# HengyiWang/MorpheuS

Hardware: AMD Instinct MI355X
Metric: rays/sec (fwd+bwd, 128 samples/ray) (higher is better)
Workload: dtype f32 (exact 3 x bf16 operand split on the bf16 MFMA pipe, fp32 accumulate)

## Files before the change

include/morpheus_hip.h:

```cpp
#ifndef MORPHEUS_HIP_H
#define MORPHEUS_HIP_H

#include <stdint.h>

#ifdef __cplusplus
extern "C" {
#endif

#define MH_OK 0
#define MH_ERR_ARG 1
#define MH_ERR_LAUNCH 2
#define MH_ERR_OVERFLOW 3

#define MH_ABI_VERSION 9
#define MH_MAX_LEVELS 32
#define MH_TILE 32

int mh_abi_version(void);
const char *mh_status_string(int status);

int mh_grid_encode_fwd(const float *x, const float *emb, const int32_t *offsets_host,
                       const int32_t *res_host, float *out, int64_t M, int32_t L, int32_t n_levels,
                       float bound, int32_t group, void *stream);
int mh_grid_encode_bwd(const float *grad, const float *x, const float *emb,
                       const int32_t *offsets_host, const int32_t *res_host, float *grad_emb,
                       float *grad_x, int64_t M, int32_t L, int32_t n_levels, float bound, void *stream);

int64_t mh_grid_bin_workspace_ints(void);
int32_t mh_grid_bin_bricks(void);
int32_t mh_grid_bin_index_ints(void);
int mh_grid_bin_points(const float *x, int64_t M, float bound, int32_t *workspace, int32_t *perm,
                       int32_t *brick_start, void *stream);
int mh_grid_encode_bwd_binned(const float *grad, const float *x, const float *emb,
                              const int32_t *offsets_host, const int32_t *res_host, const int32_t *perm,
                              const int32_t *brick_start, float *grad_emb, int64_t *emb_acc, float *grad_x, int32_t accumulate_dx,
                              int64_t M, int32_t L, int32_t n_levels, float bound, const uint32_t *gmax_bits, void *stream);
int mh_grid_encode_fwd_binned(const float *x, const float *emb, const int32_t *offsets_host, const int32_t *res_host,
                              const int32_t *perm, const int32_t *brick_start, float *out, int64_t M, int32_t L,
                              int32_t n_levels, float bound, void *stream);
int64_t mh_grid_stage_min_points(int64_t set);
int mh_grid_bwd_layout(const int32_t *res_host, int32_t L, int32_t *cbase, int32_t *stride, int32_t *rows);

int mh_grid_general_fwd(const float *x, const float *emb, const int32_t *offsets_host, const int32_t *res_host, float *out,
                        int64_t M, int32_t L, int32_t n_levels, int32_t C, int32_t gridtype, int32_t align_corners,
                        int32_t interp, float bound, void *stream);
int mh_grid_general_bwd(const float *grad, const float *x, const float *emb, const int32_t *offsets_host,
                        const int32_t *res_host, float *grad_emb, int64_t *emb_acc, float *grad_x, int64_t M, int32_t L,
                        int32_t n_levels, int32_t C, int32_t gridtype, int32_t align_corners, int32_t interp, float bound,
                        void *stream);
int mh_grid_grad_tv(const float *x, const float *emb, const int32_t *offsets_host, const int32_t *res_host, float *grad_emb,
                    int64_t *emb_acc, float weight, int64_t M, int32_t L, int32_t C, int32_t gridtype, int32_t align_corners,
                    int32_t normalized, float bound, void *stream);
int mh_grid_grad_wd(const float *emb, const int32_t *offsets_host, float *grad_emb, float weight, int32_t L, int32_t C,
                    void *stream);

int mh_composite_fwd(const float *sigma, const float *t_starts, const float *t_ends, const float *rgb,
                     const int32_t *ray_start, const int32_t *ray_cnt, float *weights, float *opacity,
                     float *depth, float *color, int32_t N, void *stream);
int mh_composite_bwd(const float *sigma, const float *t_starts, const float *t_ends, const float *rgb,
                     const int32_t *ray_start, const int32_t *ray_cnt, const float *weights,
                     const float *g_weights, const float *g_opacity, const float *g_depth,
                     const float *g_color, float *d_sigma, float *d_rgb, int32_t N, void *stream);

int mh_generate_rays(float fx, float fy, float cx, float cy, const float *c2w_host, int32_t H, int32_t W,
                     float *rays_o, float *rays_d, void *stream);
int mh_sample_uniform(const float *rays_o, const float *rays_d, const float *jitter, int32_t N, int32_t S,
                      float bound, int32_t *ray_idx, float *t_starts, float *t_ends, float *xyz,
                      int32_t *ray_start, int32_t *ray_cnt, void *stream);

int mh_rays_sample_uniform(float fx, float fy, float cx, float cy, const float *c2w_host, int32_t H, int32_t W,
                           const int32_t *pix, const float *jitter, int32_t N, int32_t S, float bound,
                           float *rays_o, float *rays_d, int32_t *ray_idx, float *t_starts, float *t_ends,
                           float *xyz, int32_t *ray_start, int32_t *ray_cnt, void *stream);

int32_t mh_march_cap(float step, float bound);
int mh_march_slots(const float *rays_o, const float *rays_d, const float *jitter, int32_t N, float step, float bound,
                   int32_t R, const uint8_t *binary, int32_t cap, int32_t *ray_cnt, float *slot_ts, float *slot_te,
                   int32_t *overflow, void *stream);
int mh_march_pack(const int32_t *ray_start, const int32_t *ray_cnt, const float *slot_ts, const float *slot_te, int32_t N,
                  int32_t cap, int32_t *ray_idx, float *t_starts, float *t_ends, void *stream);

int mh_visibility_mask(const float *values, int32_t alpha_form, const float *t_starts, const float *t_ends,
                       const int32_t *ray_start, const int32_t *ray_cnt, int32_t N, int64_t M, float early_stop_eps,
                       const float *alpha_thre, uint8_t *keep, int32_t *kept_cnt, void *stream);
int mh_visibility_pack(const uint8_t *keep, const float *t_starts, const float *t_ends, const int32_t *ray_start,
                       const int32_t *ray_cnt, const int32_t *new_start, int32_t N, int64_t M, int64_t M_out,
                       int32_t *out_ray_idx, float *out_t_starts, float *out_t_ends, int32_t *src_index, void *stream);

int mh_fd_taps(const float *x, const float *topo, int32_t topo_dim, float eps, float bound, int64_t M, float *taps,
               float *topo6, void *stream);
int mh_fd_taps_bwd(const float *x, const float *g_taps, const float *g_topo6, int32_t topo_dim, float eps, float bound,
                   int64_t M, float *g_x, float *g_topo, void *stream);
int mh_fd_normal_fwd(const float *sdf6, float eps, int64_t M, float *normal, float *raw, void *stream);
int mh_fd_normal_bwd(const float *sdf6, const float *g_normal, const float *g_raw, float eps, int64_t M, float *g_sdf6,
                     void *stream);
int mh_sample_positions(const float *rays_o, const float *rays_d, const int32_t *ray_idx, const float *t_starts,
                        const float *t_ends, int64_t M, float *xyz, void *stream);
int mh_multicode_fwd(const float *t, const float *v0, const float *v1, const float *v2, int32_t s0, int32_t s1, int32_t s2,
                     int32_t C, int32_t F, float *out, void *stream);
int mh_multicode_bwd(const float *t, const float *g_out, float *g0, float *g1, float *g2, int32_t s0, int32_t s1, int32_t s2,
                     int32_t C, int32_t F, void *stream);
int mh_sdf_losses_fwd(const float *pred_sdf, const float *t_starts, const float *t_ends, const int32_t *ray_idx,
                      const float *rays_depth, const float *rays_mask, float trunc, int64_t M, const int32_t *n_valid,
                      float *sums, void *stream);
int mh_sdf_losses_bwd(const float *pred_sdf, const float *t_starts, const float *t_ends, const int32_t *ray_idx,
                      const float *rays_depth, const float *rays_mask, float trunc, int64_t M, const int32_t *n_valid,
                      const float *sums, const float *g_fs, const float *g_sl, float *g_pred, void *stream);
int mh_sample_positions_bwd(const float *g_xyz, const float *t_starts, const float *t_ends, const int32_t *ray_start,
                            const int32_t *ray_cnt, int32_t N, float *g_o, float *g_d, void *stream);

int64_t mh_mlp_tiles(int64_t M);
int64_t mh_warp_acts_floats(int64_t M);
int64_t mh_warp_dpre_floats(int64_t M);
int64_t mh_warp_wpack_floats(void);
int64_t mh_warp_wpackT_floats(void);
int mh_warp_fwd(const float *x, const int32_t *slot, const float *bias0_d, const float *bias0_t,
                const float *wpack_d, const float *wpack_t, const float *bias_d, const float *bias_t,
                int32_t n_bands, float *out_deform, float *out_topo, float *acts, int64_t M, void *stream);
int64_t mh_field_w3_bytes(void);
int mh_field_fwd_b3(const float *xc, const float *feat_s, const float *feat_c, const float *topo, const void *w3,
                    const float *bias, const float *beta, int32_t n_bands, int32_t with_color, float *sdf, float *sigma,
                    float *albedo, float *acts, int64_t M, void *stream);
// ... 274 lines not shown
```

morpheus_amd/csrc/hashgrid.hip:

```cpp
#include "common.h"
#include "wave.h"
#include <stdlib.h>
#include <algorithm>
#include <atomic>
#include <cmath>

#pragma clang fp contract(off)

struct GridMeta {
    int32_t offsets[MH_MAX_LEVELS + 1];
    int32_t res[MH_MAX_LEVELS];
};

struct Corner8 {
    uint32_t row[8];
    float w[8];
};

__device__ __forceinline__ uint32_t grid_row(uint32_t cx, uint32_t cy, uint32_t cz, uint32_t res, uint32_t T,
                                             bool dense, bool pow2) {
    uint32_t idx;
    if (dense) {
        idx = cx + cy * res + cz * res * res;
        return idx;
// ... 280 lines not shown
    const int t = threadIdx.x;
    int32_t *work_start = brick_start + NBRK + 2;
    int loc[PER], locw[PER], s = 0, sw = 0;
#pragma unroll
    for (int k = 0; k < PER; k++) {
        const int i = t * PER + k;
        loc[k] = i <= NBRK ? brick_cnt[i] : 0;
        locw[k] = i < NBRK ? (loc[k] + chunk - 1) / chunk : 0;
        s += loc[k];
        sw += locw[k];
    }
    part[t] = s;
    partw[t] = sw;
    __syncthreads();
    for (int o = 1; o < 1024; o <<= 1) {
        const int v = t >= o ? part[t - o] : 0;
        const int vw = t >= o ? partw[t - o] : 0;
        __syncthreads();
        part[t] += v;
        partw[t] += vw;
        __syncthreads();
    }
    int run = part[t] - s, runw = partw[t] - sw;
#pragma unroll
    for (int k = 0; k < PER; k++) {
        const int i = t * PER + k;
        if (i <= NBRK) {
            brick_start[i] = run;
            work_start[i] = runw;
        }
        run += loc[k];
        runw += locw[k];
    }
    if (t == 1023) brick_start[NBRK + 1] = part[1023], brick_start[BRK_CHUNK_WORD] = chunk;
}

__global__ __launch_bounds__(256) void bin_scatter_kernel(const float *__restrict__ x, int64_t M, int64_t chunk, float bound,
                                                          float two_bound, const int32_t *__restrict__ block_off,
                                                          const int32_t *__restrict__ brick_start, int32_t *__restrict__ perm) {
    __shared__ int cur[NBRK + 1];
    for (int i = threadIdx.x; i <= NBRK; i += 256) cur[i] = brick_start[i] + block_off[(int64_t)blockIdx.x * (NBRK + 1) + i];
    __syncthreads();
    const int64_t p0 = (int64_t)blockIdx.x * chunk, p1 = min(p0 + chunk, M);
    for (int64_t p = p0 + threadIdx.x; p < p1; p += 256) {
        const int slot = atomicAdd(&cur[brick_of(x, p, bound, two_bound)], 1);
        perm[slot] = (int32_t)p;
    }
}

__global__ __launch_bounds__(256) void absmax_kernel(const float *__restrict__ g, int64_t n, uint32_t *__restrict__ out) {
    uint32_t m = 0;
    const int64_t stride = (int64_t)gridDim.x * blockDim.x;
    const int64_t n4 = n >> 2;
    const f32x4 *g4 = reinterpret_cast<const f32x4 *>(g);
    for (int64_t i = (int64_t)blockIdx.x * blockDim.x + threadIdx.x; i < n4; i += stride) {
        const f32x4 v = g4[i];
        m = max(max(m, __float_as_uint(fabsf(v[0]))), __float_as_uint(fabsf(v[1])));
        m = max(max(m, __float_as_uint(fabsf(v[2]))), __float_as_uint(fabsf(v[3])));
    }
    for (int64_t i = 4 * n4 + (int64_t)blockIdx.x * blockDim.x + threadIdx.x; i < n; i += stride) m = max(m, __float_as_uint(fabsf(g[i])));
    m = wave_max(m);
    if ((threadIdx.x & 63) == 0 && m) atomicMax(out, m);
}

#define FX_BITS 40
#define FX_MAGIC 6755399441055744.0
#define FX_MAGIC_BITS 0x4338000000000000ULL
#define FX_LIMIT 1099511627776.0f
__device__ __forceinline__ void fx_scales(uint32_t maxbits, float &to_fx, float &from_fx) {
    int e = (int)(maxbits >> 23) + 1;
    e = max(e, 60);
    e = min(e, 254);
    to_fx = __uint_as_float((uint32_t)(127 + FX_BITS + 127 - e) << 23);
    from_fx = __uint_as_float((uint32_t)(127 - FX_BITS - 127 + e) << 23);
}

#define BRK_THREADS 1024
constexpr int BRK_PIPE = 2;
constexpr int BRK_STAGE = 1;
constexpr int BRK_STAGE_UNROLL = 8;
constexpr int BRK_STAGE_MIN_POINTS = 1 << 20;
constexpr int BRK_STAGE_MIN = 96;

__device__ __forceinline__ int brk_div(int j, int m) { return (int)(((uint32_t)j * (uint32_t)m) >> 16); }

__device__ __forceinline__ bool brk_find_item(const int32_t *__restrict__ brick_start, int w, int *item) {
    const int32_t *work_start = brick_start + NBRK + 2;
    constexpr int PER = NBRK / BRK_THREADS;
    const int b0 = PER * (int)threadIdx.x;
    int ws[PER + 1], bs[PER + 1];
    const int chunk = brick_start[BRK_CHUNK_WORD];
#pragma unroll
    for (int k = 0; k <= PER; k++) ws[k] = work_start[b0 + k], bs[k] = brick_start[b0 + k];
    bool mine = false;
#pragma unroll
    for (int k = 0; k < PER; k++)
        if (ws[k] <= w && w < ws[k + 1]) {
            const int first = bs[k] + (w - ws[k]) * chunk;
            item[0] = b0 + k, item[1] = first, item[2] = min(first + chunk, bs[k + 1]), mine = true;
        }
    return __syncthreads_or(mine) != 0;
}

struct BrickLevel {
    uint32_t res, T, my, mz, mask, sel;
    bool dense, pow2;
    int nn, base, lo[3];
    const float2 *tab;
};

__device__ __forceinline__ BrickLevel brk_level(const GridMeta &meta, const BrickMeta &bm, const float2 *__restrict__ emb, int l,
                                                int brick) {
    BrickLevel v;
    v.res = (uint32_t)meta.res[l];
    v.T = (uint32_t)(meta.offsets[l + 1] - meta.offsets[l]);
    v.dense = (uint64_t)v.res * v.res * v.res <= (uint64_t)v.T;
    v.pow2 = (v.T & (v.T - 1)) == 0;
    v.my = v.dense ? v.res : 2654435761u, v.mz = v.dense ? v.res * v.res : 805459861u;
    v.mask = v.pow2 ? v.T - 1 : 0xffffffffu, v.sel = v.dense ? 0xffffffffu : 0u;
    v.nn = bm.n[l], v.base = bm.lds_off[l];
    const int bxyz[3] = {brick % BRK, (brick / BRK) % BRK, brick / (BRK * BRK)};
#pragma unroll
    for (int d = 0; d < 3; d++) {
        const float pos = fminf(fmaxf(fmaf((float)bxyz[d] / (float)BRK, (float)v.res, -0.5f), 0.0f), (float)(v.res - 1));
        v.lo[d] = (int)floorf(pos);
    }
    v.tab = emb + meta.offsets[l];
    return v;
}

template <bool ZERO>
__device__ __forceinline__ void brk_stage_rows(const BrickLevel &v, int sub, char *lds, int row0, int stride, int z0 = 0, int z1 = 0) {
    const int n3 = v.nn * v.nn * v.nn, m = (65536 + v.nn - 1) / v.nn;
    for (int j0 = sub; j0 < n3; j0 += 64 * BRK_STAGE_UNROLL) {
        float2 r[BRK_STAGE_UNROLL];
#pragma unroll
        for (int u = 0; u < BRK_STAGE_UNROLL; u++) {
            const int j = min(j0 + 64 * u, n3 - 1);
            const int t = brk_div(j, m), jz = brk_div(t, m);
            const int jx = j - t * v.nn, jy = t - jz * v.nn;
            const uint32_t cx = min((uint32_t)(v.lo[0] + jx), v.res - 1), ym = min((uint32_t)(v.lo[1] + jy), v.res - 1) * v.my,
                           zm = min((uint32_t)(v.lo[2] + jz), v.res - 1) * v.mz;
            uint32_t row = ((cx + ym + zm) & v.sel) | ((cx ^ ym ^ zm) & v.mask & ~v.sel);
            if (__builtin_expect(!v.dense && !v.pow2, 0)) row %= v.T;
            r[u] = v.tab[row];
        }
#pragma unroll
        for (int u = 0; u < BRK_STAGE_UNROLL; u++) {
            const int j = j0 + 64 * u;
            if (j < n3) {
                *reinterpret_cast<float2 *>(lds + row0 + j * stride) = r[u];
                if (ZERO) *reinterpret_cast<long long *>(lds + z0 + j * stride) = 0, *reinterpret_cast<long long *>(lds + z1 + j * stride) = 0;
            }
        }
    }
}

__device__ __forceinline__ void brk_zero_sums(int n3, int sub, char *lds, int stride, int z0, int z1) {
    for (int j = sub; j < n3; j += 64)
        *reinterpret_cast<long long *>(lds + z0 + j * stride) = 0, *reinterpret_cast<long long *>(lds + z1 + j * stride) = 0;
}

__global__ __launch_bounds__(BRK_THREADS, 8) void grid_fwd_brick_kernel(const float *__restrict__ x, const float2 *__restrict__ emb,
                                                                         GridMeta meta, BrickMeta bm,
                                                                         const int32_t *__restrict__ perm,
                                                                         const int32_t *__restrict__ brick_start,
                                                                         float2 *__restrict__ out, int L, int n_levels, float bound,
                                                                         float two_bound) {
    __shared__ long long val[BRK_NODES_MAX];
    __shared__ int item[3];
    const int l = threadIdx.x & 15, sub = threadIdx.x >> 4;
    constexpr int PPI = BRK_THREADS / 16;
    if (!brk_find_item(brick_start, blockIdx.x, item)) {
        const int s = (int)blockIdx.x - brick_start[NBRK + 2 + NBRK];
        const int first = brick_start[NBRK] + s * BRK_CHUNK_SMALL, stop = min(first + BRK_CHUNK_SMALL, brick_start[NBRK + 1]);
        for (int i = first + sub; i < stop; i += PPI) out[(int64_t)perm[i] * L + l] = make_float2(0.f, 0.f);
        return;
    }
    const int brick = item[0], start = item[1], end = item[2];
    const bool lev_on = l < n_levels;
    const BrickLevel lv = brk_level(meta, bm, emb, l, brick);
    if (lev_on) brk_stage_rows<false>(lv, sub, reinterpret_cast<char *>(val), 8 * lv.base, 8);
    __syncthreads();
    const int last = end - 1;
    int p_cur = perm[min(start + sub, last)], p_nxt = perm[min(start + sub + PPI, last)];
    float xv[3] = {x[(int64_t)p_cur * 3 + 0], x[(int64_t)p_cur * 3 + 1], x[(int64_t)p_cur * 3 + 2]};
    for (int i = start + sub; i < end; i += PPI) {
        const int p_nn = perm[min(i + 2 * PPI, last)];
        const float xn[3] = {x[(int64_t)p_nxt * 3 + 0], x[(int64_t)p_nxt * 3 + 1], x[(int64_t)p_nxt * 3 + 2]};
        float2 r = make_float2(0.f, 0.f);
        if (lev_on) {
            uint32_t g[3];
            float f[3];
            grid_locate(xv, bound, two_bound, lv.res, g, f);
            const uint32_t g1[3] = {min(g[0] + 1, lv.res - 1), min(g[1] + 1, lv.res - 1), min(g[2] + 1, lv.res - 1)};
            const int lx[2] = {(int)g[0] - lv.lo[0], (int)g1[0] - lv.lo[0]}, ly[2] = {(int)g[1] - lv.lo[1], (int)g1[1] - lv.lo[1]},
                      lz[2] = {(int)g[2] - lv.lo[2], (int)g1[2] - lv.lo[2]};
            float2 v[8];
#pragma unroll
            for (int c = 0; c < 8; c++)
                v[c] = *reinterpret_cast<const float2 *>(
                    &val[lv.base + lx[c & 1] + __mul24(lv.nn, ly[(c >> 1) & 1] + __mul24(lv.nn, lz[(c >> 2) & 1]))]);
#pragma unroll
            for (int c = 0; c < 8; c++) {
                const float w = ((c & 1) ? f[0] : 1.f - f[0]) * ((c & 2) ? f[1] : 1.f - f[1]) * ((c & 4) ? f[2] : 1.f - f[2]);
                r.x = fmaf(w, v[c].x, r.x);
                r.y = fmaf(w, v[c].y, r.y);
            }
        }
        out[(int64_t)p_cur * L + l] = r;
        p_cur = p_nxt, p_nxt = p_nn;
        xv[0] = xn[0], xv[1] = xn[1], xv[2] = xn[2];
    }
}

template <int NEED_DX, bool STAGED>
__global__ __launch_bounds__(BRK_THREADS, STAGED ? 4 : 8) void grid_bwd_brick_kernel(
    const float2 *__restrict__ grad, const float *__restrict__ x, const float2 *__restrict__ emb, GridMeta meta, BrickMeta bm,
    const int32_t *__restrict__ perm, const int32_t *__restrict__ brick_start, long long *__restrict__ emb_acc, int acc_shift,
    float *__restrict__ grad_x, int L, int n_levels, float bound, float two_bound, const uint32_t *__restrict__ gmax_bits) {
    constexpr int ACC_WORDS = STAGED ? 16 * BRK_ACC_ROWS : 2 * BRK_NODES_MAX;
    __shared__ long long acc[ACC_WORDS];
    char *accb = reinterpret_cast<char *>(acc);
    __shared__ int item[3];
    if (!brk_find_item(brick_start, blockIdx.x, item)) return;
    const int brick = item[0], start = item[1], end = item[2];
    const bool staged = STAGED && end - start >= BRK_STAGE_MIN;
    if (!STAGED)
        for (int i = threadIdx.x; i < BRK_NODES_MAX; i += BRK_THREADS) acc[2 * i] = 0, acc[2 * i + 1] = 0;
    float to_fx, from_fx;
    fx_scales(*gmax_bits, to_fx, from_fx);
    to_fx = ldexpf(to_fx, -acc_shift);
    const float fx_lim = ldexpf(FX_LIMIT, -acc_shift);
    const int l = threadIdx.x & 15, sub = threadIdx.x >> 4;
    const bool lev_on = l < n_levels;
    const BrickLevel lv = brk_level(meta, bm, emb, l, brick);
    const uint32_t res = lv.res, T = lv.T;
    const bool dense = lv.dense, pow2 = lv.pow2;
    const int nn = lv.nn, base = lv.base;
    const int lo[3] = {lv.lo[0], lv.lo[1], lv.lo[2]};
    const float2 *tab = lv.tab;
    const int stride = STAGED ? bm.stride : 16;
    const int cb0 = STAGED ? bm.cbase[0][l] : 16 * base, cb1 = STAGED ? bm.cbase[1][l] : cb0 + 8, cb2 = STAGED ? bm.cbase[2][l] : 0;
    const int d1 = cb1 - cb0, d2 = cb2 - cb0;
    if (STAGED && lev_on) {
        if (staged) brk_stage_rows<true>(lv, sub, accb, cb2, stride, cb0, cb1);
        else brk_zero_sums(nn * nn * nn, sub, accb, stride, cb0, cb1);
    }
    static_assert(MH_MAX_LEVELS >= 16, "the brick kernels run on 16-level grids (L == 16 is checked by the launchers)");
    __shared__ int flush_par[16][16];
    if (threadIdx.x < 16) {
        int *fp = flush_par[l];
        fp[0] = nn, fp[1] = (65536 + nn - 1) / nn, fp[2] = base, fp[3] = lo[0], fp[4] = lo[1], fp[5] = lo[2];
        fp[6] = (int)(res - 1), fp[7] = (int)lv.my, fp[8] = (int)lv.mz, fp[9] = (int)lv.mask, fp[10] = (int)lv.sel, fp[11] = (int)T;
        fp[12] = (int)(!dense && !pow2), fp[13] = meta.offsets[l], fp[14] = cb0, fp[15] = cb1;
    }
    __syncthreads();
    constexpr int PPI = BRK_THREADS / 16;
    const int end_r = start + ((end - start + PPI - 1) / PPI) * PPI;
    int magic_hi, magic_lo;
    asm("s_mov_b32 %0, 0x43380000" : "=s"(magic_hi));
    asm("s_mov_b32 %0, 0" : "=s"(magic_lo));
    const double magic = __longlong_as_double(((long long)magic_hi << 32) | (unsigned)magic_lo);
    const int last = end - 1;
    constexpr int PIPE = (NEED_DX && !STAGED) ? 0 : BRK_PIPE;
    int p_cur = 0, p_nxt = 0;
    float xv[3] = {0.f, 0.f, 0.f};
    float2 gr = make_float2(0.f, 0.f);
    if (PIPE == 2) {
        p_cur = perm[min(start + sub, last)];
        p_nxt = perm[min(start + sub + PPI, last)];
#pragma unroll
        for (int d = 0; d < 3; d++) xv[d] = x[(int64_t)p_cur * 3 + d];
        gr = grad[(int64_t)p_cur * L + l];
    }
    const float inv_2b = 1.0f / two_bound;
    for (int i = start + sub; i < end_r; i += PPI) {
        const bool live = i < end;
        if (PIPE == 0) p_cur = perm[min(i, last)];
        const int64_t p = p_cur;
        int p_nn = 0;
        float xn[3] = {0.f, 0.f, 0.f};
        float2 grn = make_float2(0.f, 0.f);
        if (PIPE == 2) {
            p_nn = perm[min(i + 2 * PPI, last)];
#pragma unroll
            for (int d = 0; d < 3; d++) xn[d] = x[(int64_t)p_nxt * 3 + d];
            grn = grad[(int64_t)p_nxt * L + l];
        } else {
#pragma unroll
            for (int d = 0; d < 3; d++) xv[d] = x[p * 3 + d];
            gr = grad[p * L + l];
        }
        float gx_old[3] = {0.f, 0.f, 0.f};
        if (NEED_DX == 2 && l == 0) {
#pragma unroll
            for (int d = 0; d < 3; d++) gx_old[d] = grad_x[p * 3 + d];
        }
        float dx[3] = {0.f, 0.f, 0.f};
        if (live && lev_on) {
            uint32_t g[3];
            float f[3];
            grid_locate(xv, bound, two_bound, res, g, f);
            const uint32_t g1[3] = {min(g[0] + 1, res - 1), min(g[1] + 1, res - 1), min(g[2] + 1, res - 1)};
            const int lx0 = (int)g[0] - lo[0], ly0 = (int)g[1] - lo[1], lz0 = (int)g[2] - lo[2];
            const int lx1 = (int)g1[0] - lo[0], ly1 = (int)g1[1] - lo[1], lz1 = (int)g1[2] - lo[2];
            const double gxd = (double)__builtin_amdgcn_fmed3f(gr.x * to_fx, -fx_lim, fx_lim),
                         gyd = (double)__builtin_amdgcn_fmed3f(gr.y * to_fx, -fx_lim, fx_lim);
            int slot[8];
#pragma unroll
            for (int c = 0; c < 8; c++) {
                const float w = ((c & 1) ? f[0] : 1.f - f[0]) * ((c & 2) ? f[1] : 1.f - f[1]) * ((c & 4) ? f[2] : 1.f - f[2]);
                const int li = ((c & 1) ? lx1 : lx0) + __mul24(nn, ((c & 2) ? ly1 : ly0) + __mul24(nn, (c & 4) ? lz1 : lz0));
                slot[c] = cb0 + __mul24(li, stride);
                const double wd = (double)w;
                const unsigned long long qx = (unsigned long long)__double_as_longlong(__builtin_fma(wd, gxd, magic)) - FX_MAGIC_BITS;
                const unsigned long long qy = (unsigned long long)__double_as_longlong(__builtin_fma(wd, gyd, magic)) - FX_MAGIC_BITS;
                atomicAdd(reinterpret_cast<unsigned long long *>(accb + slot[c]), qx);
                atomicAdd(reinterpret_cast<unsigned long long *>(accb + slot[c] + d1), qy);
            }
            if (NEED_DX) {
                float2 v[8];
                if (staged) {
#pragma unroll
                    for (int c = 0; c < 8; c++) v[c] = *reinterpret_cast<const float2 *>(accb + slot[c] + d2);
                } else {
                    uint32_t row[8];
                    grid_rows8(g, g1, res, T, dense, pow2, row);
#pragma unroll
                    for (int c = 0; c < 8; c++) v[c] = tab[row[c]];
                }
                grid_ddx(v, f, gr, (float)res, dx);
            }
        }
        if (NEED_DX) {
            const float sx = sum16(dx[0]), sy = sum16(dx[1]), sz = sum16(dx[2]);
            if (live && l == 0) {
                grad_x[p * 3 + 0] = gx_old[0] + sx * inv_2b;
                grad_x[p * 3 + 1] = gx_old[1] + sy * inv_2b;
                grad_x[p * 3 + 2] = gx_old[2] + sz * inv_2b;
            }
        }
        if (PIPE == 2) {
            p_cur = p_nxt, p_nxt = p_nn;
            xv[0] = xn[0], xv[1] = xn[1], xv[2] = xn[2], gr = grn;
        }
    }
    __syncthreads();
    {
        int total = 0;
        if (n_levels > 0) {
            const int n_last = bm.n[n_levels - 1];
            total = bm.lds_off[n_levels - 1] + n_last * n_last * n_last;
        }
        for (int j = threadIdx.x; j < total; j += BRK_THREADS) {
            int lev = 0;
            if (STAGED) {
#pragma unroll
                for (int k = 1; k < 16; k++) lev += (k < n_levels && j >= bm.lds_off[k]) ? 1 : 0;
            }
            const int a0 = STAGED ? flush_par[lev][14] + (j - flush_par[lev][2]) * stride : 16 * j;
            const int a1 = STAGED ? flush_par[lev][15] + (j - flush_par[lev][2]) * stride : 16 * j + 8;
            const long long qx = *reinterpret_cast<const long long *>(accb + a0), qy = *reinterpret_cast<const long long *>(accb + a1);
            if (qx == 0 && qy == 0) continue;
            if (!STAGED) {
#pragma unroll
                for (int k = 1; k < 16; k++) lev += (k < n_levels && j >= bm.lds_off[k]) ? 1 : 0;
            }
            const int *fp = flush_par[lev];
            const int n = fp[0], m = fp[1], jl = j - fp[2];
            const int t = brk_div(jl, m), jz = brk_div(t, m);
            const int jx = jl - t * n, jy = t - jz * n;
            const uint32_t rmax = (uint32_t)fp[6];
            const uint32_t cx = min((uint32_t)(fp[3] + jx), rmax), ym = min((uint32_t)(fp[4] + jy), rmax) * (uint32_t)fp[7],
                           zm = min((uint32_t)(fp[5] + jz), rmax) * (uint32_t)fp[8];
            const uint32_t sel = (uint32_t)fp[10];
            uint32_t row = ((cx + ym + zm) & sel) | ((cx ^ ym ^ zm) & (uint32_t)fp[9] & ~sel);
            if (__builtin_expect(fp[12] != 0, 0)) row %= (uint32_t)fp[11];
            unsigned long long *ga = reinterpret_cast<unsigned long long *>(emb_acc + ((size_t)fp[13] + row) * 2);
            atomicAdd(ga + 0, (unsigned long long)qx);
            atomicAdd(ga + 1, (unsigned long long)qy);
        }
    }
}

__global__ void grid_acc_finalize_kernel(const long long *__restrict__ emb_acc, float *__restrict__ grad_emb, int64_t n, int acc_shift,
                                         const uint32_t *__restrict__ gmax_bits) {
    float to_fx, from_fx;
    fx_scales(*gmax_bits, to_fx, from_fx);
    const double scale = (double)from_fx * (double)(1LL << acc_shift);
    for (int64_t i = (int64_t)blockIdx.x * blockDim.x + threadIdx.x; i < n; i += (int64_t)gridDim.x * blockDim.x) {
        const long long a = emb_acc[i];
        if (a != 0) grad_emb[i] += (float)((double)a * scale);
    }
}

static int fill_meta(GridMeta &m, const int32_t *offsets_host, const int32_t *res_host, int L) {
    if (!offsets_host || !res_host || L < 1 || L > MH_MAX_LEVELS) return MH_ERR_ARG;
    for (int i = 0; i <= L; i++) m.offsets[i] = offsets_host[i];
    for (int i = 0; i < L; i++) {
        m.res[i] = res_host[i];
        if (res_host[i] < 2 || offsets_host[i + 1] <= offsets_host[i]) return MH_ERR_ARG;
    }
    return MH_OK;
}

extern "C" int mh_grid_encode_fwd(const float *x, const float *emb, const int32_t *offsets_host,
                                  const int32_t *res_host, float *out, int64_t M, int32_t L, int32_t n_levels,
                                  float bound, int32_t group, void *stream) {
    if (M == 0) return MH_OK;
    if (!x || !emb || !out || M < 0 || n_levels < 0 || n_levels > L || !(bound > 0.f) || group < 1) return MH_ERR_ARG;
    GridMeta meta;
    int st = fill_meta(meta, offsets_host, res_host, L);
    if (st) return st;
    if (group == 6 && M % 6 == 0) {
        const int64_t n_groups = M / 6;
        const int64_t gblocks = (n_groups * L + 255) / 256;
        if (gblocks > 0x7fffffffLL) return MH_ERR_ARG;
        hipLaunchKernelGGL(grid_fwd_grouped_kernel<6>, dim3((unsigned)gblocks), dim3(256), 0, mh_stream(stream), x,
                           reinterpret_cast<const float2 *>(emb), meta, reinterpret_cast<float2 *>(out), n_groups, (int)L,
                           (int)n_levels, bound, 2.0f * bound);
        MH_CHECK_LAUNCH();
        return MH_OK;
    }
    const int64_t threads = M * L;
    const int64_t blocks = (threads + 255) / 256;
    if (blocks > 0x7fffffffLL) return MH_ERR_ARG;
    hipLaunchKernelGGL(grid_fwd_kernel, dim3((unsigned)blocks), dim3(256), 0, mh_stream(stream), x,
                       reinterpret_cast<const float2 *>(emb), meta, reinterpret_cast<float2 *>(out), M, (int)L, (int)n_levels,
                       bound, 2.0f * bound);
    MH_CHECK_LAUNCH();
    return MH_OK;
}

extern "C" int mh_grid_encode_bwd(const float *grad, const float *x, const float *emb, const int32_t *offsets_host,
                                  const int32_t *res_host, float *grad_emb, float *grad_x, int64_t M, int32_t L,
                                  int32_t n_levels, float bound, void *stream) {
    if (M == 0) return MH_OK;
    if (!grad || !x || !emb || !grad_emb || M < 0 || n_levels < 0 || n_levels > L || !(bound > 0.f)) return MH_ERR_ARG;
    if (grad_x && L != 16) return MH_ERR_ARG;
    GridMeta meta;
    int st = fill_meta(meta, offsets_host, res_host, L);
    if (st) return st;
    const int64_t threads = M * L;
    const int64_t blocks = (threads + 255) / 256;
    if (blocks > 0x7fffffffLL) return MH_ERR_ARG;
    if (grad_x)
        hipLaunchKernelGGL(grid_bwd_kernel<true>, dim3((unsigned)blocks), dim3(256), 0, mh_stream(stream),
                           reinterpret_cast<const float2 *>(grad), x, reinterpret_cast<const float2 *>(emb), meta,
                           grad_emb, grad_x, M, (int)L, (int)n_levels, bound, 2.0f * bound);
    else
        hipLaunchKernelGGL(grid_bwd_kernel<false>, dim3((unsigned)blocks), dim3(256), 0, mh_stream(stream),
                           reinterpret_cast<const float2 *>(grad), x, reinterpret_cast<const float2 *>(emb), meta,
                           grad_emb, grad_x, M, (int)L, (int)n_levels, bound, 2.0f * bound);
    MH_CHECK_LAUNCH();
// ... 19 lines not shown
    G = G < 8 ? 8 : (G > BIN_BLOCKS ? BIN_BLOCKS : G);
    const int64_t chunk = (M + G - 1) / G;
    int32_t *block_hist = workspace, *brick_cnt = workspace + (int64_t)BIN_BLOCKS * (NBRK + 1);
    hipLaunchKernelGGL(bin_hist_kernel, dim3((unsigned)G), dim3(256), 0, mh_stream(stream), x, M, chunk, bound, 2.0f * bound,
                       block_hist);
    hipLaunchKernelGGL(bin_colscan_kernel, dim3((NBRK + 1 + 255) / 256), dim3(256), 0, mh_stream(stream), block_hist,
                       (int)G, brick_cnt);
    hipLaunchKernelGGL(bin_rowscan_kernel, dim3(1), dim3(1024), 0, mh_stream(stream), brick_cnt, brick_start,
                       M >= g_stage_min_points.load(std::memory_order_relaxed) ? BRK_CHUNK_LARGE : BRK_CHUNK_SMALL);
    hipLaunchKernelGGL(bin_scatter_kernel, dim3((unsigned)G), dim3(256), 0, mh_stream(stream), x, M, chunk, bound,
                       2.0f * bound, block_hist, brick_start, perm);
    MH_CHECK_LAUNCH();
    return MH_OK;
}

static int fill_brick_meta(BrickMeta &bm, const int32_t *res_host, int L) {
    bm = BrickMeta{};
    int off = 0;
    for (int l = 0; l < L; l++) {
        const int n = (res_host[l] + BRK - 1) / BRK + 2;
        bm.n[l] = n;
        bm.lds_off[l] = off;
        off += n * n * n;
    }
    return off > BRK_NODES_MAX ? MH_ERR_ARG : MH_OK;
}

static int brick_layout_linear(BrickMeta &bm) {
    for (int k = 0; k < 3; k++)
        for (int l = 0; l < 16; l++) bm.cbase[k][l] = 8 * (3 * bm.lds_off[l] + k);
    bm.stride = 24;
    return (24 * (bm.lds_off[15] + bm.n[15] * bm.n[15] * bm.n[15]) + 127) / 128;
}

static int brick_layout(BrickMeta &bm) {
    int sz[16], col[3][16], h[16] = {}, order[48];
    bool used[3][16] = {};
    for (int l = 0; l < 16; l++) sz[l] = bm.n[l] * bm.n[l] * bm.n[l];
    for (int i = 0; i < 48; i++) order[i] = i;
    std::stable_sort(order, order + 48, [&](int a, int b) { return sz[a % 16] > sz[b % 16]; });
    for (int i = 0; i < 48; i++) {
        const int k = order[i] / 16, l = order[i] % 16;
        int best = -1;
        for (int c = 0; c < 16; c++)
            if (!used[k][c] && (best < 0 || h[c] < h[best])) best = c;
        used[k][best] = true, col[k][l] = best, h[best] += sz[l];
    }
    for (bool moved = true; moved;) {
        moved = false;
        for (int k = 0; k < 3; k++)
            for (int a = 0; a < 16; a++)
                for (int b = a + 1; b < 16; b++) {
                    const int ca = col[k][a], cb = col[k][b], d = sz[a] - sz[b];
                    if (std::max(h[ca] - d, h[cb] + d) < std::max(h[ca], h[cb]))
                        h[ca] -= d, h[cb] += d, col[k][a] = cb, col[k][b] = ca, moved = true;
                }
    }
    const int rows = *std::max_element(h, h + 16);
    if (rows > BRK_ACC_ROWS) return brick_layout_linear(bm);
    int top[16] = {};
    for (int k = 0; k < 3; k++)
        for (int l = 0; l < 16; l++) {
            const int c = col[k][l];
            bm.cbase[k][l] = 128 * top[c] + 8 * c;
            top[c] += sz[l];
        }
    bm.stride = 128;
    return rows;
}

extern "C" int mh_grid_bwd_layout(const int32_t *res_host, int32_t L, int32_t *cbase, int32_t *stride, int32_t *rows) {
    if (!res_host || !cbase || !stride || !rows || L != 16) return MH_ERR_ARG;
    for (int l = 0; l < L; l++)
        if (res_host[l] < 2) return MH_ERR_ARG;
    BrickMeta bm;
    if (int st = fill_brick_meta(bm, res_host, L)) return st;
    *rows = brick_layout(bm);
    *stride = bm.stride;
    for (int k = 0; k < 3; k++)
        for (int l = 0; l < 16; l++) cbase[16 * k + l] = bm.cbase[k][l];
    return MH_OK;
}

extern "C" int mh_grid_encode_fwd_binned(const float *x, const float *emb, const int32_t *offsets_host,
                                         const int32_t *res_host, const int32_t *perm, const int32_t *brick_start, float *out,
                                         int64_t M, int32_t L, int32_t n_levels, float bound, void *stream) {
    if (M == 0) return MH_OK;
    if (!x || !emb || !out || !perm || !brick_start || M < 0 || M > 0x7fffffffLL || n_levels < 0 || n_levels > L || L != 16 ||
        !(bound > 0.f))
        return MH_ERR_ARG;
    GridMeta meta;
    int st = fill_meta(meta, offsets_host, res_host, L);
    if (st) return st;
    BrickMeta bm;
    if ((st = fill_brick_meta(bm, res_host, L))) return st;
    const unsigned work_items = (unsigned)(NBRK + M / BRK_CHUNK_SMALL + 1);
    hipLaunchKernelGGL(grid_fwd_brick_kernel, dim3(work_items), dim3(BRK_THREADS), 0, mh_stream(stream), x,
                       reinterpret_cast<const float2 *>(emb), meta, bm, perm, brick_start, reinterpret_cast<float2 *>(out), (int)L,
                       (int)n_levels, bound, 2.0f * bound);
    MH_CHECK_LAUNCH();
    return MH_OK;
}

extern "C" int mh_grid_encode_bwd_binned(const float *grad, const float *x, const float *emb, const int32_t *offsets_host,
                                         const int32_t *res_host, const int32_t *perm, const int32_t *brick_start,
                                         float *grad_emb, int64_t *emb_acc, float *grad_x, int32_t accumulate_dx, int64_t M,
                                         int32_t L, int32_t n_levels, float bound, const uint32_t *gmax_bits, void *stream) {
    if (M == 0) return MH_OK;
    if (!grad || !x || !emb || !grad_emb || !emb_acc || !perm || !brick_start || M < 0 || n_levels < 0 || n_levels > L || L != 16 ||
        !(bound > 0.f))
        return MH_ERR_ARG;
    GridMeta meta;
    int st = fill_meta(meta, offsets_host, res_host, L);
    if (st) return st;
    BrickMeta bm;
    if ((st = fill_brick_meta(bm, res_host, L))) return st;
    const bool staged = BRK_STAGE && grad_x && M >= g_stage_min_points.load(std::memory_order_relaxed);
    if (staged) brick_layout(bm);
    const unsigned work_items = (unsigned)(NBRK + M / BRK_CHUNK_SMALL + 1);
    int acc_shift = 0;
    while (acc_shift < 40 && (double)M * 8.0 > std::ldexp(1.0, 62 - FX_BITS + acc_shift)) acc_shift++;
    const int64_t n_acc = (int64_t)offsets_host[L] * 2;
    if (!mh_zero_async(emb_acc, sizeof(int64_t) * (size_t)n_acc, mh_stream(stream))) return MH_ERR_LAUNCH;
    const uint32_t *gmax = gmax_bits;
    if (!gmax) {
        uint32_t *own = reinterpret_cast<uint32_t *>(const_cast<int32_t *>(brick_start)) + (2 * NBRK + 4);
        if (!mh_zero_async(own, sizeof(uint32_t), mh_stream(stream))) return MH_ERR_LAUNCH;
        hipLaunchKernelGGL(absmax_kernel, dim3(1024), dim3(256), 0, mh_stream(stream), grad, M * (int64_t)L * 2, own);
        gmax = own;
    }
#define BRK_LAUNCH(DXMODE, STG)                                                                                                \
    hipLaunchKernelGGL((grid_bwd_brick_kernel<DXMODE, STG>), dim3(work_items), dim3(BRK_THREADS), 0, mh_stream(stream),       \
                       reinterpret_cast<const float2 *>(grad), x, reinterpret_cast<const float2 *>(emb), meta, bm, perm,     \
                       brick_start, reinterpret_cast<long long *>(emb_acc), acc_shift, grad_x, (int)L, (int)n_levels, bound,          \
                       2.0f * bound, gmax)
    if (grad_x && accumulate_dx) {
        if (staged) BRK_LAUNCH(2, true); else BRK_LAUNCH(2, false);
    } else if (grad_x) {
        if (!mh_zero_async(grad_x, sizeof(float) * 3 * (size_t)M, mh_stream(stream))) return MH_ERR_LAUNCH;
        if (staged) BRK_LAUNCH(1, true); else BRK_LAUNCH(1, false);
    } else {
        BRK_LAUNCH(0, false);
    }
#undef BRK_LAUNCH
    MH_CHECK_LAUNCH();
    hipLaunchKernelGGL(grid_acc_finalize_kernel, dim3((unsigned)std::min<int64_t>((n_acc + 255) / 256, 4096)), dim3(256), 0,
                       mh_stream(stream), reinterpret_cast<const long long *>(emb_acc), grad_emb, n_acc, acc_shift, gmax);
    MH_CHECK_LAUNCH();
    return MH_OK;
}
```

morpheus_amd/ops.py:

```python
from __future__ import annotations

import ctypes
import math
import os
from typing import Optional, Sequence

import numpy as np
import torch

from . import _lib
from ._lib import check, launch, ptr, require_gpu, stream
from .packing import field_joint_packer, field_packer, warp_joint_packer, warp_packer



class KernelTimer:

    def __init__(self):
        self.enabled = False
        self.records = {}
        self._pool, self._used = [], 0

    def reset(self, enabled: bool):
        self.enabled, self.records, self._used = enabled, {}, 0
# ... 56 lines not shown
            key = (len(a),) + tuple(int(v) for v in a)
            hit = _I32_CACHE.get(key)
            if hit is None:
                arr = np.ascontiguousarray(a, dtype=np.int32)
                arr.setflags(write=False)
                hit = _I32_CACHE[key] = (arr, arr.ctypes.data_as(ctypes.c_void_p))
            _I32_CACHE[k2] = hit
            return hit
        key = None
    elif isinstance(a, np.ndarray) and a.dtype == np.int32 and a.ndim == 1 and a.size <= 64:
        key = (a.size,) + tuple(a.tolist())
    else:
        key = None
    if key is not None:
        hit = _I32_CACHE.get(key)
        if hit is None:
            arr = np.ascontiguousarray(a, dtype=np.int32)
            arr.setflags(write=False)
            hit = _I32_CACHE[key] = (arr, arr.ctypes.data_as(ctypes.c_void_p))
        return hit
    a = np.ascontiguousarray(a, dtype=np.int32)
    return a, a.ctypes.data_as(ctypes.c_void_p)


def _scratch(n: int, device, dtype=torch.float32) -> torch.Tensor:
    n = int(n)
    if n >= (1 << 18):
        q = 1 << (n.bit_length() - 4)
        return torch.empty((n + q - 1) // q * q, dtype=dtype, device=device)[:n]
    return torch.empty(n, dtype=dtype, device=device)


def level_resolutions(L: int, per_level_scale: float, base: int) -> np.ndarray:
    S = np.float32(np.log2(per_level_scale))
    l = np.arange(L, dtype=np.float32)
    return np.ceil(np.exp2(l * S).astype(np.float32) * np.float32(base)).astype(np.int32)


def effective_levels(max_level, L: int) -> int:
    return L if max_level is None else max(min(int(math.ceil(max_level * L)), L), 1)


def _bin_points(lib, x, bound):
    M, dev = x.shape[0], x.device
    ws = torch.empty(lib.mh_grid_bin_workspace_ints(), dtype=torch.int32, device=dev)
    perm = _scratch(M, dev, torch.int32)
    bstart = torch.empty(lib.mh_grid_bin_index_ints(), dtype=torch.int32, device=dev)
    _timed("mh_grid_bin_points", ptr(x), M, bound, ptr(ws), ptr(perm), ptr(bstart))
    return perm, bstart


MLP_MODES = ("b3", "f32")
MODE_DTYPE = {"f32": "f32", "b3": "f32 (exact 3 x bf16 operand split, 6 slice products per MAC on the bf16 MFMA pipe, fp32 accumulate)"}
_mode = os.environ.get("MORPHEUS_MLP", "b3")
if _mode not in MLP_MODES:
    raise ValueError(f"MORPHEUS_MLP={_mode!r}: expected one of {MLP_MODES}")


def mlp_mode() -> str:
    return _mode


def set_mlp_mode(mode: str) -> str:
    global _mode
    if mode not in MLP_MODES:
        raise ValueError(f"mlp mode {mode!r}: expected one of {MLP_MODES}")
    prev, _mode = _mode, mode
    return prev


def _warp_mode(mode: Optional[str] = None) -> str:
    mode = _mode if mode is None else mode
    if mode not in MLP_MODES:
        raise ValueError(f"mlp mode {mode!r}: expected one of {MLP_MODES}")
    return "" if mode == "f32" else mode


def _grid_fwd(lib, x, embs, o_p, r_p, L, n_levels, bound, group):
    M = x.shape[0]
    outs = []
    binned = None
    if L == 16 and M >= lib.mh_grid_stage_min_points(-1):
        binned = _bin_points(lib, x, bound)
    for emb in embs:
        out = _scratch(M * L * 2, x.device).view(M, L * 2)
        if binned is not None:
            _timed("mh_grid_encode_fwd_binned", ptr(x), ptr(emb), o_p, r_p, ptr(binned[0]), ptr(binned[1]), ptr(out), M, L,
                   n_levels, float(bound))
        else:
            _timed("mh_grid_encode_fwd", ptr(x), ptr(emb), o_p, r_p, ptr(out), M, L, n_levels, float(bound), int(group))
        outs.append(out)
    return outs, binned


def _grid_bwd(lib, x, embs, grads, o_p, r_p, L, n_levels, bound, need_dx, gmax_ptrs=None, sums=None, g_x_into=None, binned=None):
    M = x.shape[0]
    g_x_total, g_embs = g_x_into, []
    brick = M > 0 and L == 16
    for k, (emb, grad) in enumerate(zip(embs, grads)):
        if grad is None:
            g_embs.append(None)
            continue
        grad = grad.contiguous()
        into = None if sums is None else sums[k]
        g_emb = torch.zeros_like(emb) if into is None else None
        g_emb_p = ptr(g_emb) if into is None else ctypes.c_void_p(into)
        if brick:
            if binned is None:
                binned = _bin_points(lib, x, bound)
            acc_dx = need_dx and g_x_total is not None
            g_x = g_x_total if acc_dx else (torch.empty_like(x) if need_dx else None)
            emb_acc = torch.empty(emb.numel(), dtype=torch.int64, device=emb.device)
            _timed("mh_grid_encode_bwd_binned", ptr(grad), ptr(x), ptr(emb), o_p, r_p, ptr(binned[0]), ptr(binned[1]), g_emb_p,
                   ptr(emb_acc), ptr(g_x), int(acc_dx), M, L, n_levels, bound, None if gmax_ptrs is None else gmax_ptrs[k])
            g_x_total = g_x
        else:
            g_x = torch.empty_like(x) if need_dx else None
            _timed("mh_grid_encode_bwd", ptr(grad), ptr(x), ptr(emb), o_p, r_p, g_emb_p, ptr(g_x), M, L, n_levels, bound)
            if need_dx:
                g_x_total = g_x if g_x_total is None else g_x_total + g_x
        g_embs.append(g_emb)
    return (g_x_total if need_dx else None), g_embs


class _GridEncode(torch.autograd.Function):

    @staticmethod
    def forward(ctx, x, offsets_np, res_np, n_levels, bound, group, *embs):
        ctx.set_materialize_grads(False)
        require_gpu(x, *embs)
        lib = _lib.load()
        x = x.detach().contiguous().float()
        L = len(res_np)
        o_np, o_p = _i32arr(offsets_np)
        r_np, r_p = _i32arr(res_np)
        saved = [emb.detach().contiguous() for emb in embs]
        outs, ctx.binned = _grid_fwd(lib, x, saved, o_p, r_p, L, n_levels, bound, group)
        ctx.save_for_backward(x, *saved)
        ctx.meta = (o_np, r_np, n_levels, float(bound), L)
        return tuple(outs)

    @staticmethod
    def backward(ctx, *grads):
        lib = _lib.load()
        x, *embs = ctx.saved_tensors
        o_np, r_np, n_levels, bound, L = ctx.meta
        o_p, r_p = o_np.ctypes.data_as(ctypes.c_void_p), r_np.ctypes.data_as(ctypes.c_void_p)
        g_x, g_embs = _grid_bwd(lib, x, embs, grads, o_p, r_p, L, n_levels, bound, ctx.needs_input_grad[0], binned=ctx.binned)
        return (g_x, None, None, None, None, None, *g_embs)


def grid_encode(x, emb, offsets_np, res_np, bound, max_level=None, group: int = 1):
    L = len(res_np)
    lead = list(x.shape[:-1])
    (out,) = _GridEncode.apply(x.reshape(-1, 3), offsets_np, res_np, effective_levels(max_level, L), bound, group, emb)
    return out.view(lead + [L * 2])


def grid_encode_multi(x, embs, offsets_np, res_np, bound, max_level=None):
    L = len(res_np)
    return _GridEncode.apply(x.reshape(-1, 3), offsets_np, res_np, effective_levels(max_level, L), bound, 1, *embs)


GRID_TYPES = {"hash": 0, "tiled": 1}
GRID_INTERPS = {"linear": 0, "smoothstep": 1}
GRID_CHANNELS = (1, 2, 4, 8)
# ... 1561 lines not shown
```

Measured before the change: 1.103 million.

## Fuse two hash-grid tables into one binned forward brick kernel launch

Adds a paired forward brick kernel that stages both embedding tables into LDS side by side, interleaved per node as 16-byte entries. Each point then reads one 16-byte vector per corner and interpolates both outputs in a single pass. This shares the binning lookup, point loads and per-corner index math across the two tables and removes a second launch. It also swaps several index multiplies for 24-bit mul intrinsics. Costs are doubled LDS per block, which may reduce occupancy, and a fallback to two launches when the tables are too large for 32-bit byte offsets.

```diff
diff --git a/include/morpheus_hip.h b/include/morpheus_hip.h
--- a/include/morpheus_hip.h
+++ b/include/morpheus_hip.h
@@ -38,6 +38,9 @@
 int mh_grid_encode_fwd_binned(const float *x, const float *emb, const int32_t *offsets_host, const int32_t *res_host,
                               const int32_t *perm, const int32_t *brick_start, float *out, int64_t M, int32_t L,
                               int32_t n_levels, float bound, void *stream);
+int mh_grid_encode_fwd_binned2(const float *x, const float *emb0, const float *emb1, const int32_t *offsets_host,
+                               const int32_t *res_host, const int32_t *perm, const int32_t *brick_start, float *out0,
+                               float *out1, int64_t M, int32_t L, int32_t n_levels, float bound, void *stream);
 int64_t mh_grid_stage_min_points(int64_t set);
 int mh_grid_bwd_layout(const int32_t *res_host, int32_t L, int32_t *cbase, int32_t *stride, int32_t *rows);
 
diff --git a/morpheus_amd/csrc/hashgrid.hip b/morpheus_amd/csrc/hashgrid.hip
--- a/morpheus_amd/csrc/hashgrid.hip
+++ b/morpheus_amd/csrc/hashgrid.hip
@@ -386,7 +386,7 @@
 constexpr int BRK_STAGE_MIN_POINTS = 1 << 20;
 constexpr int BRK_STAGE_MIN = 96;
 
-__device__ __forceinline__ int brk_div(int j, int m) { return (int)(((uint32_t)j * (uint32_t)m) >> 16); }
+__device__ __forceinline__ int brk_div(int j, int m) { return (int)(__umul24((uint32_t)j, (uint32_t)m) >> 16); }
 
 __device__ __forceinline__ bool brk_find_item(const int32_t *__restrict__ brick_start, int w, int *item) {
     const int32_t *work_start = brick_start + NBRK + 2;
@@ -433,27 +433,36 @@
     return v;
 }
 
-template <bool ZERO>
-__device__ __forceinline__ void brk_stage_rows(const BrickLevel &v, int sub, char *lds, int row0, int stride, int z0 = 0, int z1 = 0) {
+template <bool ZERO, int NT = 1>
+__device__ __forceinline__ void brk_stage_rows(const BrickLevel &v, int sub, char *lds, int row0, int stride, int z0 = 0, int z1 = 0,
+                                               const float2 *__restrict__ emb0 = nullptr, const float2 *__restrict__ emb1 = nullptr,
+                                               uint32_t row_l = 0, int row1 = 0) {
     const int n3 = v.nn * v.nn * v.nn, m = (65536 + v.nn - 1) / v.nn;
     for (int j0 = sub; j0 < n3; j0 += 64 * BRK_STAGE_UNROLL) {
-        float2 r[BRK_STAGE_UNROLL];
+        float2 r[NT][BRK_STAGE_UNROLL];
 #pragma unroll
         for (int u = 0; u < BRK_STAGE_UNROLL; u++) {
             const int j = min(j0 + 64 * u, n3 - 1);
             const int t = brk_div(j, m), jz = brk_div(t, m);
-            const int jx = j - t * v.nn, jy = t - jz * v.nn;
+            const int jx = j - __mul24(t, v.nn), jy = t - __mul24(jz, v.nn);
             const uint32_t cx = min((uint32_t)(v.lo[0] + jx), v.res - 1), ym = min((uint32_t)(v.lo[1] + jy), v.res - 1) * v.my,
                            zm = min((uint32_t)(v.lo[2] + jz), v.res - 1) * v.mz;
             uint32_t row = ((cx + ym + zm) & v.sel) | ((cx ^ ym ^ zm) & v.mask & ~v.sel);
             if (__builtin_expect(!v.dense && !v.pow2, 0)) row %= v.T;
-            r[u] = v.tab[row];
+            if (NT == 2) {
+                const uint32_t o = (row_l + row) * 8u;
+                r[0][u] = *reinterpret_cast<const float2 *>(reinterpret_cast<const char *>(emb0) + o);
+                r[NT - 1][u] = *reinterpret_cast<const float2 *>(reinterpret_cast<const char *>(emb1) + o);
+            } else {
+                r[0][u] = v.tab[row];
+            }
         }
 #pragma unroll
         for (int u = 0; u < BRK_STAGE_UNROLL; u++) {
             const int j = j0 + 64 * u;
             if (j < n3) {
-                *reinterpret_cast<float2 *>(lds + row0 + j * stride) = r[u];
+                *reinterpret_cast<float2 *>(lds + row0 + j * stride) = r[0][u];
+                if (NT == 2) *reinterpret_cast<float2 *>(lds + row1 + j * stride) = r[NT - 1][u];
                 if (ZERO) *reinterpret_cast<long long *>(lds + z0 + j * stride) = 0, *reinterpret_cast<long long *>(lds + z1 + j * stride) = 0;
             }
         }
@@ -465,34 +474,49 @@
         *reinterpret_cast<long long *>(lds + z0 + j * stride) = 0, *reinterpret_cast<long long *>(lds + z1 + j * stride) = 0;
 }
 
+template <int NT>
 __global__ __launch_bounds__(BRK_THREADS, 8) void grid_fwd_brick_kernel(const float *__restrict__ x, const float2 *__restrict__ emb,
                                                                          GridMeta meta, BrickMeta bm,
                                                                          const int32_t *__restrict__ perm,
                                                                          const int32_t *__restrict__ brick_start,
                                                                          float2 *__restrict__ out, int L, int n_levels, float bound,
-                                                                         float two_bound) {
-    __shared__ long long val[BRK_NODES_MAX];
+                                                                         float two_bound, const float2 *__restrict__ emb1,
+                                                                         float2 *__restrict__ out1) {
+    __shared__ __attribute__((aligned(16))) long long val[NT * BRK_NODES_MAX];
     __shared__ int item[3];
     const int l = threadIdx.x & 15, sub = threadIdx.x >> 4;
     constexpr int PPI = BRK_THREADS / 16;
     if (!brk_find_item(brick_start, blockIdx.x, item)) {
         const int s = (int)blockIdx.x - brick_start[NBRK + 2 + NBRK];
         const int first = brick_start[NBRK] + s * BRK_CHUNK_SMALL, stop = min(first + BRK_CHUNK_SMALL, brick_start[NBRK + 1]);
-        for (int i = first + sub; i < stop; i += PPI) out[(int64_t)perm[i] * L + l] = make_float2(0.f, 0.f);
+        for (int i = first + sub; i < stop; i += PPI) {
+            const int64_t o = (int64_t)perm[i] * L + l;
+            out[o] = make_float2(0.f, 0.f);
+            if (NT == 2) out1[o] = make_float2(0.f, 0.f);
+        }
         return;
     }
     const int brick = item[0], start = item[1], end = item[2];
     const bool lev_on = l < n_levels;
     const BrickLevel lv = brk_level(meta, bm, emb, l, brick);
-    if (lev_on) brk_stage_rows<false>(lv, sub, reinterpret_cast<char *>(val), 8 * lv.base, 8);
+    if (lev_on) {
+        if (NT == 2)
+            brk_stage_rows<false, 2>(lv, sub, reinterpret_cast<char *>(val), 16 * lv.base, 16, 0, 0, emb, emb1,
+                                     (uint32_t)meta.offsets[l], 16 * lv.base + 8);
+        else
+            brk_stage_rows<false>(lv, sub, reinterpret_cast<char *>(val), 8 * lv.base, 8);
+    }
     __syncthreads();
-    const int last = end - 1;
+    const int last = end - 1, nn2 = lv.nn * lv.nn;
     int p_cur = perm[min(start + sub, last)], p_nxt = perm[min(start + sub + PPI, last)];
     float xv[3] = {x[(int64_t)p_cur * 3 + 0], x[(int64_t)p_cur * 3 + 1], x[(int64_t)p_cur * 3 + 2]};
+    if (NT == 2) asm volatile("" : "+v"(xv[0]), "+v"(xv[1]), "+v"(xv[2]), "+v"(p_nxt));
     for (int i = start + sub; i < end; i += PPI) {
         const int p_nn = perm[min(i + 2 * PPI, last)];
         const float xn[3] = {x[(int64_t)p_nxt * 3 + 0], x[(int64_t)p_nxt * 3 + 1], x[(int64_t)p_nxt * 3 + 2]};
-        float2 r = make_float2(0.f, 0.f);
+        float2 r[NT];
+#pragma unroll
+        for (int t = 0; t < NT; t++) r[t] = make_float2(0.f, 0.f);
         if (lev_on) {
             uint32_t g[3];
             float f[3];
@@ -500,19 +524,41 @@
             const uint32_t g1[3] = {min(g[0] + 1, lv.res - 1), min(g[1] + 1, lv.res - 1), min(g[2] + 1, lv.res - 1)};
             const int lx[2] = {(int)g[0] - lv.lo[0], (int)g1[0] - lv.lo[0]}, ly[2] = {(int)g[1] - lv.lo[1], (int)g1[1] - lv.lo[1]},
                       lz[2] = {(int)g[2] - lv.lo[2], (int)g1[2] - lv.lo[2]};
-            float2 v[8];
-#pragma unroll
-            for (int c = 0; c < 8; c++)
-                v[c] = *reinterpret_cast<const float2 *>(
-                    &val[lv.base + lx[c & 1] + __mul24(lv.nn, ly[(c >> 1) & 1] + __mul24(lv.nn, lz[(c >> 2) & 1]))]);
-#pragma unroll
-            for (int c = 0; c < 8; c++) {
-                const float w = ((c & 1) ? f[0] : 1.f - f[0]) * ((c & 2) ? f[1] : 1.f - f[1]) * ((c & 4) ? f[2] : 1.f - f[2]);
-                r.x = fmaf(w, v[c].x, r.x);
-                r.y = fmaf(w, v[c].y, r.y);
-            }
-        }
-        out[(int64_t)p_cur * L + l] = r;
+            if (NT == 2) {
+                typedef float f32x2 __attribute__((ext_vector_type(2)));
+                typedef float f32x4 __attribute__((ext_vector_type(4)));
+                const int sx[2] = {lv.base + lx[0], lv.base + lx[1]}, sy[2] = {__mul24(lv.nn, ly[0]), __mul24(lv.nn, ly[1])},
+                          sz[2] = {__mul24(nn2, lz[0]), __mul24(nn2, lz[1])};
+                f32x4 q[8];
+#pragma unroll
+                for (int c = 0; c < 8; c++)
+                    q[c] = *reinterpret_cast<const f32x4 *>(&val[2 * (sx[c & 1] + (sy[(c >> 1) & 1] + sz[(c >> 2) & 1]))]);
+                f32x2 s0 = {0.f, 0.f}, s1 = {0.f, 0.f};
+#pragma unroll
+                for (int c = 0; c < 8; c++) {
+                    const float w = ((c & 1) ? f[0] : 1.f - f[0]) * ((c & 2) ? f[1] : 1.f - f[1]) * ((c & 4) ? f[2] : 1.f - f[2]);
+                    const f32x2 ww = {w, w};
+                    s0 = __builtin_elementwise_fma(ww, q[c].xy, s0);
+                    s1 = __builtin_elementwise_fma(ww, q[c].zw, s1);
+                }
+                r[0] = make_float2(s0.x, s0.y), r[NT - 1] = make_float2(s1.x, s1.y);
+            } else {
+                float2 v[8];
+#pragma unroll
+                for (int c = 0; c < 8; c++)
+                    v[c] = *reinterpret_cast<const float2 *>(
+                        &val[lv.base + lx[c & 1] + __mul24(lv.nn, ly[(c >> 1) & 1] + __mul24(lv.nn, lz[(c >> 2) & 1]))]);
+#pragma unroll
+                for (int c = 0; c < 8; c++) {
+                    const float w = ((c & 1) ? f[0] : 1.f - f[0]) * ((c & 2) ? f[1] : 1.f - f[1]) * ((c & 4) ? f[2] : 1.f - f[2]);
+                    r[0].x = fmaf(w, v[c].x, r[0].x);
+                    r[0].y = fmaf(w, v[c].y, r[0].y);
+                }
+            }
+        }
+        const int64_t o = (int64_t)p_cur * L + l;
+        out[o] = r[0];
+        if (NT == 2) out1[o] = r[NT - 1];
         p_cur = p_nxt, p_nxt = p_nn;
         xv[0] = xn[0], xv[1] = xn[1], xv[2] = xn[2];
     }
@@ -674,7 +720,7 @@
             const int *fp = flush_par[lev];
             const int n = fp[0], m = fp[1], jl = j - fp[2];
             const int t = brk_div(jl, m), jz = brk_div(t, m);
-            const int jx = jl - t * n, jy = t - jz * n;
+            const int jx = jl - __mul24(t, n), jy = t - __mul24(jz, n);
             const uint32_t rmax = (uint32_t)fp[6];
             const uint32_t cx = min((uint32_t)(fp[3] + jx), rmax), ym = min((uint32_t)(fp[4] + jy), rmax) * (uint32_t)fp[7],
                            zm = min((uint32_t)(fp[5] + jz), rmax) * (uint32_t)fp[8];
@@ -860,24 +906,51 @@
     return MH_OK;
 }
 
-extern "C" int mh_grid_encode_fwd_binned(const float *x, const float *emb, const int32_t *offsets_host,
-                                         const int32_t *res_host, const int32_t *perm, const int32_t *brick_start, float *out,
-                                         int64_t M, int32_t L, int32_t n_levels, float bound, void *stream) {
+static int grid_fwd_binned(const float *x, const float *emb, const float *emb1, const int32_t *offsets_host, const int32_t *res_host,
+                           const int32_t *perm, const int32_t *brick_start, float *out, float *out1, bool pair, int64_t M,
+                           int32_t L, int32_t n_levels, float bound, void *stream) {
     if (M == 0) return MH_OK;
     if (!x || !emb || !out || !perm || !brick_start || M < 0 || M > 0x7fffffffLL || n_levels < 0 || n_levels > L || L != 16 ||
         !(bound > 0.f))
         return MH_ERR_ARG;
+    if (pair && (!emb1 || !out1 || out1 == out)) return MH_ERR_ARG;
     GridMeta meta;
     int st = fill_meta(meta, offsets_host, res_host, L);
     if (st) return st;
     BrickMeta bm;
     if ((st = fill_brick_meta(bm, res_host, L))) return st;
     const unsigned work_items = (unsigned)(NBRK + M / BRK_CHUNK_SMALL + 1);
-    hipLaunchKernelGGL(grid_fwd_brick_kernel, dim3(work_items), dim3(BRK_THREADS), 0, mh_stream(stream), x,
-                       reinterpret_cast<const float2 *>(emb), meta, bm, perm, brick_start, reinterpret_cast<float2 *>(out), (int)L,
-                       (int)n_levels, bound, 2.0f * bound);
+    if (pair && offsets_host[L] >= (1 << 28)) {
+        for (int t = 0; t < 2; t++)
+            hipLaunchKernelGGL(grid_fwd_brick_kernel<1>, dim3(work_items), dim3(BRK_THREADS), 0, mh_stream(stream), x,
+                               reinterpret_cast<const float2 *>(t ? emb1 : emb), meta, bm, perm, brick_start,
+                               reinterpret_cast<float2 *>(t ? out1 : out), (int)L, (int)n_levels, bound, 2.0f * bound,
+                               (const float2 *)nullptr, (float2 *)nullptr);
+    } else if (pair)
+        hipLaunchKernelGGL(grid_fwd_brick_kernel<2>, dim3(work_items), dim3(BRK_THREADS), 0, mh_stream(stream), x,
+                           reinterpret_cast<const float2 *>(emb), meta, bm, perm, brick_start, reinterpret_cast<float2 *>(out),
+                           (int)L, (int)n_levels, bound, 2.0f * bound, reinterpret_cast<const float2 *>(emb1),
+                           reinterpret_cast<float2 *>(out1));
+    else
+        hipLaunchKernelGGL(grid_fwd_brick_kernel<1>, dim3(work_items), dim3(BRK_THREADS), 0, mh_stream(stream), x,
+                           reinterpret_cast<const float2 *>(emb), meta, bm, perm, brick_start, reinterpret_cast<float2 *>(out),
+                           (int)L, (int)n_levels, bound, 2.0f * bound, (const float2 *)nullptr, (float2 *)nullptr);
     MH_CHECK_LAUNCH();
     return MH_OK;
+}
+
+extern "C" int mh_grid_encode_fwd_binned(const float *x, const float *emb, const int32_t *offsets_host,
+                                         const int32_t *res_host, const int32_t *perm, const int32_t *brick_start, float *out,
+                                         int64_t M, int32_t L, int32_t n_levels, float bound, void *stream) {
+    return grid_fwd_binned(x, emb, nullptr, offsets_host, res_host, perm, brick_start, out, nullptr, false, M, L, n_levels, bound,
+                           stream);
+}
+
+extern "C" int mh_grid_encode_fwd_binned2(const float *x, const float *emb0, const float *emb1, const int32_t *offsets_host,
+                                          const int32_t *res_host, const int32_t *perm, const int32_t *brick_start, float *out0,
+                                          float *out1, int64_t M, int32_t L, int32_t n_levels, float bound, void *stream) {
+    return grid_fwd_binned(x, emb0, emb1, offsets_host, res_host, perm, brick_start, out0, out1, true, M, L, n_levels, bound,
+                           stream);
 }
 
 extern "C" int mh_grid_encode_bwd_binned(const float *grad, const float *x, const float *emb, const int32_t *offsets_host,
diff --git a/morpheus_amd/ops.py b/morpheus_amd/ops.py
--- a/morpheus_amd/ops.py
+++ b/morpheus_amd/ops.py
@@ -162,6 +162,11 @@
     binned = None
     if L == 16 and M >= lib.mh_grid_stage_min_points(-1):
         binned = _bin_points(lib, x, bound)
+        if len(embs) == 2:
+            outs = [_scratch(M * L * 2, x.device).view(M, L * 2) for _ in embs]
+            _timed("mh_grid_encode_fwd_binned2", ptr(x), ptr(embs[0]), ptr(embs[1]), o_p, r_p, ptr(binned[0]), ptr(binned[1]),
+                   ptr(outs[0]), ptr(outs[1]), M, L, n_levels, float(bound), key="mh_grid_encode_fwd_binned")
+            return outs, binned
     for emb in embs:
         out = _scratch(M * L * 2, x.device).view(M, L * 2)
         if binned is not None:
```

Measured after the change: 1.112 million, median of 6. About the same (+0.8%).
